# nextpyp/cet_pick

Measured on AMD Instinct MI355X. Metric: subtomograms/sec (MoCo-3D train) + voxels/sec (heatmap+NMS) at 1/2/4/8 GPU, higher is better.
Workload: dtype f32; 1 GPU; moco_main.py moco3d_18: 3D encoder, synthetic 512x512x128 tomogram, 32^3 subtomo crops, batch 64 per GPU, r=1024, dim=128, m=0.999, T=0.1, SGD lr 1e-3; global_batch=64, parallelism=dp1, hipgraph=True

## Files before the change

### cet_pick_amd/_lib.py

```python
import ctypes
import os

import torch

_HERE = os.path.dirname(os.path.abspath(__file__))
LIB_PATH = os.environ.get("CETPICK_HIP_LIB") or os.path.join(_HERE, "libcetpick_hip.so")

_c = ctypes
_P, _I, _F, _Z, _D, _L = _c.c_void_p, _c.c_int, _c.c_float, _c.c_size_t, _c.c_double, _c.c_long


class ConvGeom(ctypes.Structure):
    _fields_ = [(f, _I) for f in "N Di Hi Wi Ci Co kd kh kw stride pd ph pw dd dh dw".split()]


_G = _c.POINTER(ConvGeom)


class Aug2d3dRanges(ctypes.Structure):
    _fields_ = [(f, _F) for f in "flip_p angle_lo angle_hi erase_p scale_lo scale_hi ratio_lo ratio_hi".split()]


_R = _c.POINTER(Aug2d3dRanges)

# ... 10 lines not shown
    _fields_ = [(f, _I) for f in "P M R T label_dx label_dy glyph_px glyph_gap box_pad box_border".split()]


_PL = _c.POINTER(PlotLayout)

SIGNATURES = {
    "mi_abi_version": (_I, []),
    "mi_graph_node_counts": (_I, [_P, _P]),
    "mi_debug_stamp": (_I, [_P, _P]),
    "mi_linear_stats_fwd_f32": (_I, [_P] * 5 + [_I] * 3 + [_P]),
    "mi_debug_last_conv_kernel": (_c.c_char_p, []),
    "mi_debug_last_conv_plan": (_I, [_P, _I]),
    "mi_linear_bn_fwd_f32": (_I, [_P] * 5 + [_I] * 3 + [_P, _P, _F, _F] + [_P] * 4 + [_I, _P]),
    "mi_conv3d_stem_stats_workspace_bytes": (_Z, [_I] * 5),
    "mi_conv3d_stem_stats_f32": (_I, [_P, _P, _P] + [_I] * 5 + [_P, _P, _Z, _P]),
    "mi_build_arch": (_c.c_char_p, []),
    "mi_sigmoid_clamp": (_I, [_P, _P, _Z, _P]),
    "mi_nms3d": (_I, [_P, _P, _I, _I, _I, _I, _I, _P]),
    "mi_decode_workspace_bytes": (_Z, [_I, _I, _I, _I]),
    "mi_decode_workspace_init": (_I, [_P, _Z, _P]),
    "mi_sigmoid_nms_topk": (_I, [_P, _P, _I, _I, _I, _I, _I, _I, _I, _P, _P, _P, _Z, _P]),
    "mi_gauss3d_sep": (_I, [_P, _P, _P, _I, _I, _I, _F, _P]),
    "mi_dog_pick_workspace_bytes": (_Z, [_I, _I, _I, _I]),
    "mi_dog_pick": (_I, [_P, _I, _I, _I, _P, _I, _I, _I, _I, _P, _P, _P, _P, _I, _P, _P, _Z, _P]),
    "mi_greedy_nms3d_workspace_bytes": (_Z, [_I, _I, _I]),
    "mi_greedy_nms3d": (_I, [_P, _I, _I, _I, _F, _F, _F, _P, _P, _P, _I, _P, _Z, _P]),
    "mi_crop_normalize": (_I, [_P, _I, _I, _I, _P, _I, _I, _I, _I, _I, _I, _P, _P]),
    "mi_crop_normalize_table": (_I, [_P, _P, _P, _P, _P, _c.c_int64, _I, _I, _I, _I, _I, _I, _P, _P]),
    "mi_u8_roundtrip_normalize": (_I, [_P, _P, _Z, _F, _F, _P]),
    "mi_aug2d_params": (_I, [_P, _c.c_int64, _c.c_uint64, _I, _I, _I] + [_F] * 7 + [_P, _P]),
# ... 253 lines not shown
```

### cet_pick_amd/csrc/conv_igemm.hip

```cpp
#include "common.h"
#include "bf16x3.h"
#include <algorithm>
#include <cstdlib>
#include <type_traits>

int mi_stem7_fwd(const float* x, const float* w, float* y, const float* res, int relu, int N, int D, int H, int W,
                 int Co, int bf16x3, void* ws, size_t ws_bytes, hipStream_t s, double* sums = nullptr);
size_t mi_stem7_fwd_workspace_bytes();
size_t mi_stem7_fwd_stats_workspace_bytes(int N, int D, int H, int W);
size_t mi_stem7_wgrad_workspace_bytes(int N, int D, int H, int W, int Co);
int mi_stem7_wgrad(const float* x, const float* dy, float* dw, int N, int D, int H, int W, int Co, int bf16x3, void* ws,
                   size_t ws_bytes, hipStream_t s);

int mi_direct3_kind(int N, int Di, int Hi, int Wi, int Ci, int Co, int kd, int kh, int kw, int stride, int pd, int ph,
                    int pw, int dd, int dh, int dw);
size_t mi_direct3_wimg_bytes(int channels);
size_t mi_direct3_slab_bytes(int N, int channels);
int mi_direct3_prep(const float* const* w, void* const* img, const int* dgrad, const int* channels, int n, hipStream_t s);
int mi_direct3_launch(const float* a, const void* wimg, float* out, const float* res, const float* mask, int relu, int N,
                      int D, hipStream_t s);
size_t mi_direct3_wimg_bytes_kind(int kind);
int mi_direct3_prep_kind(const float* const* w, void* const* img, const int* dgrad, const int* kinds, int n, hipStream_t s);
int mi_direct3s_launch256(const float* a, const void* wimg, float* out, const float* res, const float* mask, int relu, int N,
                          hipStream_t s);
// ... 1227 lines not shown

extern "C" size_t mi_conv3d_stem_stats_workspace_bytes(int N, int Di, int Hi, int Wi, int Co) {
    Geom g = make_geom(N, Di, Hi, Wi, 1, Co, 7, 2, 3);
    if (!geom_ok(g) || !is_stem7(g) || Co != 64) return 0;
    return mi_stem7_fwd_stats_workspace_bytes(N, Di, Hi, Wi);
}

extern "C" int mi_conv3d_stem_stats_f32(const float* x, const float* w, float* y, int N, int Di, int Hi, int Wi, int Co,
                                        double* sums, void* ws, size_t ws_bytes, mi_stream_t stream) {
    Geom g = make_geom(N, Di, Hi, Wi, 1, Co, 7, 2, 3);
    if (!x || !w || !y || !sums || !geom_ok(g)) return MI_E_ARG;
    if (!is_stem7(g) || !conv_arith_bf16x3() || env_int("MI_CONV_NO_STEM") || env_int("MI_STEM_NO_STATS")) return MI_E_UNSUPPORTED;
    return mi_stem7_fwd(x, w, y, nullptr, 0, N, Di, Hi, Wi, Co, 1, ws, ws_bytes, (hipStream_t)stream, sums);
}

extern "C" int mi_linear_fwd_f32(const float* x, const float* w, const float* bias, float* y, int M, int Ci, int Co,
                                 void* ws, size_t ws_bytes, mi_stream_t stream) {
    Geom g = make_geom(M, 1, 1, 1, Ci, Co, 1, 1, 0);
    if (!x || !w || !y || !geom_ok(g)) return MI_E_ARG;
    return run_conv(MODE_FWD, g, x, w, y, bias, nullptr, 0, ws, ws_bytes, (hipStream_t)stream, nullptr, bias ? 1 : 0);
}

extern "C" int mi_conv_wgrad_batch_f32(const float* const* xs, const float* const* dys, float* const* dws, void* const* wss, int nb,
                                       const mi_conv_geom* pg, size_t ws_bytes, int* splits_out, mi_stream_t stream) {
    Geom g;
    if (!xs || !dys || !dws || !wss || !splits_out || nb < 1 || !public_geom(pg, &g)) return MI_E_ARG;
    for (int i = 0; i < nb; ++i) if (!xs[i] || !dys[i] || !dws[i]) return MI_E_ARG;
    if (nb < 2 || !conv_arith_bf16x3() || env_int("MI_NO_WGRAD_BATCH")) return MI_E_UNSUPPORTED;
    hipStream_t s = (hipStream_t)stream;
    float* slabs[MI_WGRAD_BATCH_MAX];
// ... 82 lines not shown
```

### cet_pick_amd/csrc/conv_stem.hip

```cpp
#include "common.h"
#include "bf16x3.h"
#include <type_traits>
#include "../../include/cetpick_hip.h"

namespace {

using namespace bf3;

constexpr int K7 = 7, S2 = 2, P3 = 3;
constexpr int TX = 8, TY = 4, TZ = 4;
constexpr int PX = S2 * (TX - 1) + K7;
constexpr int PY = S2 * (TY - 1) + K7;
constexpr int PZ = S2 * (TZ - 1) + K7;
constexpr int PW = 24;
constexpr int PATCH = PZ * PY * PW;
constexpr int KS = 50;
constexpr int WS = 64;
constexpr int WROWS = 64;
constexpr int CO = 64;

struct StemParams {
    const float* x;
    const float* w;
    float* y;
    const float* res;
    int relu;
    int N, D, H, W, Do, Ho, Wo;
    unsigned x_bytes;
    double* stats;
};

__global__ __launch_bounds__(256) void stem_fwd_kernel(StemParams p) {
    constexpr int NP = (PATCH + PW + 255) / 256;
    __shared__ __attribute__((aligned(16))) float patch[NP * 256];
    __shared__ __attribute__((aligned(16))) float wl[2][WROWS * WS];
    const int tid = threadIdx.x, lane = tid & 63, wave = tid >> 6;
    const int h = lane >> 5, l32 = lane & 31;
    const int txn = p.Wo / TX, tyn = p.Ho / TY, tzn = p.Do / TZ;
    int b = blockIdx.x;
    const int bx = b % txn; b /= txn;
    const int by = b % tyn; b /= tyn;
    const int bz = b % tzn;
    const int n = b / tzn;
    const int ox0 = bx * TX, oy0 = by * TY, oz0 = bz * TZ;
// ... 93 lines not shown
constexpr int WSLAB = 3 * WPL;
constexpr size_t WPREP_BYTES = (size_t)K7 * WSLAB;

__global__ __launch_bounds__(256) void stem_wprep_kernel(const float* w, unsigned short* out) {
    const int i = blockIdx.x * 256 + threadIdx.x;
    if (i >= K7 * 8 * CO * 8) return;
    const int kx = i & 7, co = (i >> 3) & (CO - 1), j = (i >> 9) & 7, slab = i >> 12;
    const int r = 8 * slab + j, kz = r / K7, ky = r % K7;
    const float v = (r < K7 * K7 && kx < K7) ? w[((kz * K7 + ky) * K7 + kx) * CO + co] : 0.f;
    unsigned h0, h1, h2;
    cut3(v, h0, h1, h2);
    const int o = slab * (WSLAB / 2) + (j * CO + co) * 8 + kx;
    out[o] = (unsigned short)h0; out[o + WPL / 2] = (unsigned short)h1; out[o + WPL] = (unsigned short)h2;
}

template <int NBUF, int ZPW>
__global__ __launch_bounds__(256, ZPW == 2 ? 2 : (NBUF == 1 ? 3 : 2)) void stem_fwd_bf3_kernel(StemParams p, const unsigned char* wprep) {
    constexpr int TZ = 4 * ZPW;
    constexpr int PZ = S2 * (TZ - 1) + K7;
    constexpr int PPLANE = PZ * PYP * PROW;
    __shared__ __attribute__((aligned(16))) unsigned char patchb[3 * PPLANE];
    __shared__ __attribute__((aligned(16))) unsigned char wl[NBUF][WSLAB];
    const int tid = threadIdx.x, lane = tid & 63, wave = tid >> 6;
    const int h = lane >> 5, l32 = lane & 31;
    const int txn = p.Wo / TX, tyn = p.Ho / TY, tzn = p.Do / TZ;
    int b = blockIdx.x;
    const int bx = b % txn; b /= txn;
    const int by = b % tyn; b /= tyn;
    const int bz = b % tzn;
    const int n = b / tzn;
    const int ox0 = bx * TX, oy0 = by * TY, oz0 = bz * TZ;

// ... 123 lines not shown
            frags(sl + 1, 0, S0{}, nextTail);
        } else {
            frags(sl + 1, 0, S0{}, nextTail);
            __builtin_amdgcn_sched_barrier(0);
            mfmas(S1{});
        }
    };
    __syncthreads();
    frags(0, 0, S0{}, NoTail{});
    for (int sl = 0; sl < K7 - 2; ++sl) slab_body(sl, NoTail{});
    slab_body(K7 - 2, Tail{});
    __builtin_amdgcn_sched_barrier(0);
    mfmas(S0{});

    float cs[2][2];
#pragma unroll
    for (int j = 0; j < 2; ++j) {
        const int co = j * 32 + l32;
        float t0 = 0.f, t1 = 0.f;
#pragma unroll
        for (int zi = 0; zi < ZPW; ++zi) {
            const int oz = oz0 + ZPW * wave + zi;
#pragma unroll
            for (int r = 0; r < 16; ++r) {
                const int m = (r & 3) + 8 * (r >> 2) + 4 * h;
                const int ox = ox0 + (m & 7), oy = oy0 + (m >> 3);
                const long o = ((((long)n * p.Do + oz) * p.Ho + oy) * p.Wo + ox) * CO + co;
                float v = j == 0 ? acc0[zi][r] : acc1[zi][r];
                if (p.res) v += p.res[o];
                if (p.relu) v = fmaxf(v, 0.f);
                p.y[o] = v;
                t0 += v; t1 = fmaf(v, v, t1);
            }
        }
        cs[j][0] = t0; cs[j][1] = t1;
    }
    if (p.stats) {
        float* red = reinterpret_cast<float*>(patchb);
#pragma unroll
        for (int j = 0; j < 2; ++j)
#pragma unroll
            for (int q = 0; q < 2; ++q) {
                const float o = cs[j][q] + __shfl_xor(cs[j][q], 32);
                if (h == 0) red[(wave * 2 + q) * CO + j * 32 + l32] = o;
            }
        __syncthreads();
        if (tid < 2 * CO) {
            const int q = tid >> 6, c = tid & (CO - 1);
            double a = 0;
#pragma unroll
            for (int w = 0; w < 4; ++w) a += (double)red[(w * 2 + q) * CO + c];
            p.stats[(long)(q * CO + c) * gridDim.x + blockIdx.x] = a;
        }
    }
}

__global__ __launch_bounds__(256) void stem_stats_finalize_kernel(const double* part, int n_part, double* sums) {
    __shared__ double red[256];
    const double* src = part + (long)blockIdx.x * n_part;
    double a = 0;
    for (int i = threadIdx.x; i < n_part; i += 256) a += src[i];
    red[threadIdx.x] = a;
    __syncthreads();
#pragma unroll
    for (int o = 128; o > 0; o >>= 1) {
        if ((int)threadIdx.x < o) red[threadIdx.x] += red[threadIdx.x + o];
        __syncthreads();
    }
// ... 366 lines not shown
        MI_RETURN_IF_LAUNCH_FAILED();
        const bool z8 = Do % (2 * TZ) == 0 && !getenv("MI_STEM_FWD_Z4") && !getenv("MI_STEM_FWD_NBUF2");
        const long nb = z8 ? blocks / 2 : blocks;
        if (z8) hipLaunchKernelGGL((stem_fwd_bf3_kernel<1, 2>), dim3((unsigned)nb), dim3(256), 0, s, p, (const unsigned char*)ws);
        else if (getenv("MI_STEM_FWD_NBUF2")) hipLaunchKernelGGL((stem_fwd_bf3_kernel<2, 1>), dim3((unsigned)blocks), dim3(256), 0, s, p, (const unsigned char*)ws);
        else hipLaunchKernelGGL((stem_fwd_bf3_kernel<1, 1>), dim3((unsigned)blocks), dim3(256), 0, s, p, (const unsigned char*)ws);
        MI_RETURN_IF_LAUNCH_FAILED();
        if (sums) {
            hipLaunchKernelGGL(stem_stats_finalize_kernel, dim3(2 * CO), dim3(256), 0, s, (const double*)p.stats, (int)nb,
                               sums);
            MI_RETURN_IF_LAUNCH_FAILED();
        }
        return MI_OK;
    }
    hipLaunchKernelGGL(stem_fwd_kernel, dim3((unsigned)blocks), dim3(256), 0, s, p);
    MI_RETURN_IF_LAUNCH_FAILED();
    return MI_OK;
}

constexpr int RED_GROUPS = 32;

static int stem7_wgrad_blocks(long tiles) {
    long b = tiles < 512 ? tiles : 512;
    return (int)b;
}

size_t mi_stem7_wgrad_workspace_bytes(int N, int D, int H, int W, int Co) {
    if (Co != CO) return 0;
    const int Do = (D + 2 * P3 - K7) / S2 + 1, Ho = (H + 2 * P3 - K7) / S2 + 1, Wo = (W + 2 * P3 - K7) / S2 + 1;
    if (Do <= 0 || Ho <= 0 || Wo <= 0 || Do % TZ || Ho % TY || Wo % TX) return 0;
// ... 34 lines not shown
```

### cet_pick_amd/csrc/train_ops.hip

```cpp
#include "common.h"
#include "bf16x3.h"
#include <algorithm>

namespace {

using bf3::ld4;
using bf3::st4;

enum { CR_STATS = 0, CR_BNBWD = 1, CR_SUM = 2, CR_BNBWD_X = 3 };

struct PoolGeom { int N, Di, Hi, Wi, Do, Ho, Wo, k, s, pad; };

struct ColReduceParams {
    const float* a;
    const float* x;
    const float* y;
    const float* save;
    long M;
    int C, relu;
    double* partials;
    const float* gamma;
    const float* beta;
    double* sums_direct;
    float* f32_direct;
// ... 133 lines not shown
struct BnStat4 { float mean[4], inv[4]; double var[4]; };
__device__ __forceinline__ BnStat4 bn_stat4(const double* sums, double count, int C, int c, float eps) {
    BnStat4 r;
#pragma unroll
    for (int k = 0; k < 4; ++k) {
        const double mean = sums[c + k] / count;
        double var = sums[C + c + k] / count - mean * mean;
        if (var < 0) var = 0;
        r.mean[k] = (float)mean;
        r.inv[k] = (float)(1.0 / sqrt(var + (double)eps));
        r.var[k] = var;
    }
    return r;
}

__global__ __launch_bounds__(256) void bn_apply_kernel(const float* x, float* y, long n4, int C,
                                                      const double* sums, double count, float eps,
                                                      float momentum, float* running_mean,
                                                      float* running_var, long long* num_batches_tracked,
                                                      float* save, const float* gamma,
                                                      const float* beta, const float* res, int relu) {
    const int CV = C >> 2;
    const int c = (int)(threadIdx.x % CV) * 4;
    float m[4], iv[4];
    if (sums) {
        const BnStat4 st = bn_stat4(sums, count, C, c, eps);
#pragma unroll
        for (int k = 0; k < 4; ++k) { m[k] = st.mean[k]; iv[k] = st.inv[k]; }
        if (blockIdx.x == 0 && threadIdx.x < CV) {
#pragma unroll
            for (int k = 0; k < 4; ++k) {
                if (save) { save[c + k] = m[k]; save[C + c + k] = iv[k]; }
                if (running_mean) {
                    const double unbiased = count > 1 ? st.var[k] * count / (count - 1.0) : st.var[k];
                    running_mean[c + k] = (1.f - momentum) * running_mean[c + k] + momentum * m[k];
                    running_var[c + k] = (1.f - momentum) * running_var[c + k] + momentum * (float)unbiased;
                }
            }
            if (threadIdx.x == 0 && num_batches_tracked) *num_batches_tracked += 1;
        }
    } else {
#pragma unroll
        for (int k = 0; k < 4; ++k) { m[k] = running_mean[c + k]; iv[k] = 1.0f / sqrtf(running_var[c + k] + eps); }
        if (save && blockIdx.x == 0 && threadIdx.x < CV) {
#pragma unroll
            for (int k = 0; k < 4; ++k) { save[c + k] = m[k]; save[C + c + k] = iv[k]; }
        }
    }
    const float4 g = gamma ? ld4(gamma + c) : make_float4(1, 1, 1, 1);
    const float4 b = beta ? ld4(beta + c) : make_float4(0, 0, 0, 0);
    for (long i = (long)blockIdx.x * 256 + threadIdx.x; i < n4; i += (long)gridDim.x * 256) {
        float4 v = ld4(x + 4 * i);
        float4 o;
        o.x = fmaf((v.x - m[0]) * iv[0], g.x, b.x); o.y = fmaf((v.y - m[1]) * iv[1], g.y, b.y);
        o.z = fmaf((v.z - m[2]) * iv[2], g.z, b.z); o.w = fmaf((v.w - m[3]) * iv[3], g.w, b.w);
// ... 3 lines not shown
    }
}

__global__ __launch_bounds__(256) void bn_relu_maxpool_fwd_kernel(const float* x, float* y, uint8_t* arg, PoolGeom g,
                                                                 int C, const double* sums, double count, float eps,
                                                                 float momentum, float* running_mean,
                                                                 float* running_var, long long* num_batches_tracked,
                                                                 float* save, const float* gamma, const float* beta) {
    const int CV = C >> 2;
    const int c = (int)(threadIdx.x % CV) * 4;
    float m[4], iv[4];
    if (sums) {
        const BnStat4 st = bn_stat4(sums, count, C, c, eps);
#pragma unroll
        for (int k = 0; k < 4; ++k) { m[k] = st.mean[k]; iv[k] = st.inv[k]; }
        if (blockIdx.x == 0 && threadIdx.x < CV) {
#pragma unroll
            for (int k = 0; k < 4; ++k) {
                if (save) { save[c + k] = m[k]; save[C + c + k] = iv[k]; }
                if (running_mean) {
                    const double unbiased = count > 1 ? st.var[k] * count / (count - 1.0) : st.var[k];
                    running_mean[c + k] = (1.f - momentum) * running_mean[c + k] + momentum * m[k];
                    running_var[c + k] = (1.f - momentum) * running_var[c + k] + momentum * (float)unbiased;
                }
            }
            if (threadIdx.x == 0 && num_batches_tracked) *num_batches_tracked += 1;
        }
    } else {
#pragma unroll
        for (int k = 0; k < 4; ++k) { m[k] = running_mean[c + k]; iv[k] = 1.0f / sqrtf(running_var[c + k] + eps); }
    }
    const float4 g4 = gamma ? ld4(gamma + c) : make_float4(1, 1, 1, 1);
    const float4 b4 = beta ? ld4(beta + c) : make_float4(0, 0, 0, 0);
    const float gg[4] = {g4.x, g4.y, g4.z, g4.w}, bb[4] = {b4.x, b4.y, b4.z, b4.w};
    const long total = (long)g.N * g.Do * g.Ho * g.Wo * CV;
    for (long i = (long)blockIdx.x * 256 + threadIdx.x; i < total; i += (long)gridDim.x * 256) {
        unsigned v = (unsigned)i / (unsigned)CV;
        const int xo = (int)(v % (unsigned)g.Wo); v /= (unsigned)g.Wo;
        const int yo = (int)(v % (unsigned)g.Ho); v /= (unsigned)g.Ho;
        const int zo = (int)(v % (unsigned)g.Do);
        const int n = (int)(v / (unsigned)g.Do);
        float best[4] = {-INFINITY, -INFINITY, -INFINITY, -INFINITY};
// ... 39 lines not shown
                    const float4 t4 = ld4(x + ((((long)n * g.Di + zi) * g.Hi + yi) * g.Wi + xi) * C + c);
                    const float xv[4] = {t4.x, t4.y, t4.z, t4.w};
                    const int tap = (a * g.k + b) * g.k + cc;
#pragma unroll
                    for (int q = 0; q < 4; ++q) {
                        const float t = fmaxf(fmaf((xv[q] - m[q]) * iv[q], gg[q], bb[q]), 0.f);
                        const float tn = xv[q] != xv[q] ? xv[q] : t;
                        if (first || tn > best[q] || tn != tn) { best[q] = tn; bi[q] = tap; }
                    }
                    first = false;
                }
            }
        }
        st4(y + 4 * i, make_float4(best[0], best[1], best[2], best[3]));
        if (arg) *reinterpret_cast<uchar4*>(arg + 4 * i) = make_uchar4(bi[0], bi[1], bi[2], bi[3]);
    }
}

__global__ __launch_bounds__(256) void bn_relu_bwd_apply_x_kernel(const float* dy, const float* x, float* dx, long n4, int C,
                                                                 const float* save, const float* gamma, const float* beta,
                                                                 const double* sums, double count, float* dgamma,
                                                                 float* dbeta) {
    const int CV = C >> 2;
    const int c = (int)(threadIdx.x % CV) * 4;
    const float rc = (float)(1.0 / count);
    float mean[4], inv[4], gi[4], gg[4], bb[4], sdy[4], sdx[4];
#pragma unroll
    for (int k = 0; k < 4; ++k) {
        mean[k] = save[c + k]; inv[k] = save[C + c + k];
        gg[k] = gamma ? gamma[c + k] : 1.f; bb[k] = beta ? beta[c + k] : 0.f;
// ... 654 lines not shown
                                        float* running_mean, float* running_var, long long* num_batches_tracked,
                                        float* save_mean_invstd, mi_stream_t stream) {
    PoolGeom g;
    if (!x || !y || !colreduce_ok(C) || !pool_geom(N, Di, Hi, Wi, k, stride, pad, &g)) return MI_E_ARG;
    if (sums ? (!save_mean_invstd || !(count > 0)) : (!running_mean || !running_var)) return MI_E_ARG;
    if ((running_mean == nullptr) != (running_var == nullptr)) return MI_E_ARG;
    const long total = (long)N * g.Do * g.Ho * g.Wo * (C / 4);
    if (total >= (1l << 31)) return MI_E_UNSUPPORTED;
    hipLaunchKernelGGL(bn_relu_maxpool_fwd_kernel, dim3(ew_blocks(total)), dim3(256), 0, (hipStream_t)stream, x, y, argmax,
                       g, C, sums, count, eps, momentum, running_mean, running_var, num_batches_tracked,
                       save_mean_invstd, gamma, beta);
    MI_RETURN_IF_LAUNCH_FAILED();
    return MI_OK;
}

extern "C" int mi_bn_relu_bwd_reduce_x(const float* dy, const float* x, long M, int C, const float* save_mean_invstd,
                                       const float* gamma, const float* beta, double* sums, void* ws, size_t ws_bytes,
                                       mi_stream_t stream) {
    if (!dy || !x || !save_mean_invstd || !sums) return MI_E_ARG;
    ColReduceParams p = {};
    p.a = dy; p.x = x; p.save = save_mean_invstd; p.M = M; p.C = C; p.gamma = gamma; p.beta = beta;
    return run_colreduce<CR_BNBWD_X>(p, sums, ws, ws_bytes, (hipStream_t)stream);
}

extern "C" int mi_bn_relu_bwd_apply_x(const float* dy, const float* x, float* dx, long M, int C,
                                      const float* save_mean_invstd, const float* gamma, const float* beta,
                                      const double* sums, double count, float* dgamma, float* dbeta, mi_stream_t stream) {
    if (!dy || !x || !dx || !save_mean_invstd || !sums || !colreduce_ok(C) || M <= 0 || !(count > 0)) return MI_E_ARG;
    const long n4 = M * C / 4;
    hipLaunchKernelGGL(bn_relu_bwd_apply_x_kernel, dim3(ew_blocks(n4)), dim3(256), 0, (hipStream_t)stream, dy, x, dx, n4, C,
// ... 428 lines not shown
```

### cet_pick_amd/hipops.py

```python
import collections
import ctypes
import math
import os
import torch
import torch.nn as nn

from . import _lib as L


PROFILE = None
PROFILE_REPEAT = 8


def _prof_run(tag, flops, fn):
    fn()
    if PROFILE is not None:
        e0 = torch.cuda.Event(enable_timing=True)
        e1 = torch.cuda.Event(enable_timing=True)
        e0.record()
        for _ in range(PROFILE_REPEAT):
            fn()
        e1.record()
        PROFILE.append((tag, flops, e0, e1, PROFILE_REPEAT))

# ... 898 lines not shown
    if nbytes == 0:
        return None
    do, ho, wo = [(v + 6 - 7) // 2 + 1 for v in (d, h, wd)]
    y = torch.empty((n, do, ho, wo, co), dtype=torch.float32, device=x.device)
    sums = torch.empty(2 * co, dtype=torch.float64, device=x.device)
    ws = _ws(nbytes, x.device, "stem_stats")
    rc = lib.mi_conv3d_stem_stats_f32(L.ptr(x), L.ptr(w), L.ptr(y), n, d, h, wd, co, L.ptr(sums), L.ptr(ws), ws.numel(),
                                      L.stream())
    if rc == -3:
        return None
    L.check(rc, "mi_conv3d_stem_stats_f32")
    mod.bn_sums = sums
    return y


class GradSlot:
    __slots__ = ("tensor",)

    def __init__(self):
        self.tensor = None


FUSE_RES_GRAD = os.environ.get("CETPICK_FUSE_RES_GRAD", "1") != "0"


def grad_slot_for(x):
    return GradSlot() if (FUSE_RES_GRAD and torch.is_grad_enabled() and x.requires_grad and x.is_cuda and PROFILE is None) else None


class _ConvFn(torch.autograd.Function):
# ... 1483 lines not shown
```

### cet_pick_amd/models/networks/moco_encoder_3d.py

```python
import torch
import torch.nn as nn

from ... import hipops as H

BN_MOMENTUM = 0.1


def fill_fc_weights(layers):
    for m in layers.modules():
        if isinstance(m, H.HipConv3d):
            nn.init.normal_(m.weight, std=0.001)
        elif isinstance(m, H.HipLinear):
            nn.init.normal_(m.weight, std=0.001)
            if m.bias is not None:
                nn.init.constant_(m.bias, 0.001)


class BasicBlock(nn.Module):
    expansion = 1

    def __init__(self, inplanes, planes, stride=1, dilation=1, downsample=None):
        super().__init__()
        if dilation != 1:
            raise NotImplementedError("dilation != 1 is not used by the moco3d encoder")
# ... 47 lines not shown
            layers.append(block(self.inplanes, planes, dilation=dilation))
        return nn.Sequential(*layers)

    grad_marker = None

    def _mark(self, x, tag):
        if self.grad_marker is not None and x.requires_grad:
            x.register_hook(lambda g, t=tag: self.grad_marker(t))
        return x

    def _trunk(self, x1):
        b, c, d, h, w = x1.shape
        if c != 1:
            raise ValueError("the moco3d encoder takes single-channel sub-tomograms (B,1,D,H,W)")
        x = x1.contiguous().float().view(b, d, h, w, 1)
        self.conv1.stats_for_bn = self.bn1.training or not self.bn1.track_running_stats
        x = self.conv1(x)
        sums = getattr(self.conv1, "bn_sums", None) if self.conv1.stats_for_bn else None
        self.conv1.bn_sums = None
        H.stamp("stem")
        x = self._mark(H.bn_relu_maxpool3d(x, self.bn1, 3, 2, 1, sums=sums), "layer1")
        H.stamp("pool")
        first = True
        for tag, layer in (("layer2", self.layer1), ("layer3", self.layer2), (None, self.layer3)):
            for blk in layer:
                x = blk(x, mask_dx=not first, dout_masked=True)
                first = False
            if tag is not None:
                x = self._mark(x, tag)
            H.stamp("layer")
        x = self.feature_3d[0](x, mask_dx=True)
        if H.RELU_TAP is not None:
            import copy
            with torch.no_grad():
                H.RELU_TAP["feature_3d"] = copy.deepcopy(self.feature_3d[1])(x.detach(), relu=True).clone()
        x = H.bn_relu_global_avgpool(x, self.feature_3d[1])
# ... 3 lines not shown
        seq = self.__getattr__(head)
        H.stamp("trunk")
        x = H.linear_bn(x, seq[0], seq[1], relu=True)
        if H.RELU_TAP is not None:
            H.RELU_TAP[head + ".1"] = x.detach().clone()
        x = H.linear_bn(x, seq[3], seq[4], relu=True)
        if H.RELU_TAP is not None:
            H.RELU_TAP[head + ".4"] = x.detach().clone()
        return H.linear_bn(x, seq[6], seq[7])

    def forward_sync_gen(self, x1):
        b, c, d, h, w = x1.shape
        if c != 1:
            raise ValueError("the moco3d encoder takes single-channel sub-tomograms (B,1,D,H,W)")
        x = x1.contiguous().float().view(b, d, h, w, 1)
        self.conv1.stats_for_bn = True
        x = self.conv1(x)
        sums = getattr(self.conv1, "bn_sums", None)
        self.conv1.bn_sums = None
        if sums is None:
            sums = H.bn_local_sums(x)
        yield sums
        x = self._mark(H.bn_relu_maxpool3d(x, self.bn1, 3, 2, 1, sums=sums, reduced=True), "layer1")
        first = True
        for tag, layer in (("layer2", self.layer1), ("layer3", self.layer2), (None, self.layer3)):
            for blk in layer:
                x = blk(x, mask_dx=not first, dout_masked=True)
                first = False
            if tag is not None:
                x = self._mark(x, tag)
        x = self.feature_3d[0](x, mask_dx=True)
        sums = H.bn_local_sums(x)
        yield sums
        x = H.global_avgpool(self.feature_3d[1](x, relu=True, sums=sums, reduced=True))
        x = self.fc(x)
        ret1 = {}
        for head in self.heads:
            if "proj" in head:
# ... 48 lines not shown
```

### include/cetpick_hip.h

```cpp
#ifndef CETPICK_HIP_H
#define CETPICK_HIP_H

#include <stddef.h>
#include <stdint.h>

#ifdef __cplusplus
extern "C" {
#endif

typedef void* mi_stream_t;

#define MI_OK 0
#define MI_E_ARG (-1)
#define MI_E_WORKSPACE (-2)
#define MI_E_UNSUPPORTED (-3)

int mi_abi_version(void);
int mi_graph_node_counts(void* graph, int* counts);
int mi_debug_stamp(void* slot, mi_stream_t stream);
const char* mi_debug_last_conv_kernel(void);
int mi_debug_last_conv_plan(int* out, int n);
const char* mi_build_arch(void);


// ... 193 lines not shown
size_t mi_zhead_bwd_workspace_bytes(int N, int D, long P, int C, int K);
int mi_zhead_bwd(const float* x, const float* w, const float* dy, float* dx, float* dw, int N, int D, long P, int C,
                 int K, void* ws, size_t ws_bytes, mi_stream_t stream);

size_t mi_colreduce_workspace_bytes(long M, int C);
int mi_bn_stats(const float* x, long M, int C, double* sums, void* ws, size_t ws_bytes,
                mi_stream_t stream);
int mi_bn_apply_fwd(const float* x, float* y, long M, int C, const double* sums, double count,
                    const float* gamma, const float* beta, float eps, float momentum,
                    float* running_mean, float* running_var, long long* num_batches_tracked,
                    float* save_mean_invstd, const float* res, int relu, mi_stream_t stream);
int mi_bn_relu_maxpool3d_fwd(const float* x, float* y, uint8_t* argmax, int N, int Di, int Hi, int Wi, int C, int k,
                             int stride, int pad, const double* sums, double count, const float* gamma,
                             const float* beta, float eps, float momentum, float* running_mean, float* running_var,
                             long long* num_batches_tracked, float* save_mean_invstd, mi_stream_t stream);
int mi_bn_relu_bwd_reduce_x(const float* dy, const float* x, long M, int C, const float* save_mean_invstd,
                            const float* gamma, const float* beta, double* sums, void* ws, size_t ws_bytes,
                            mi_stream_t stream);
int mi_bn_relu_bwd_apply_x(const float* dy, const float* x, float* dx, long M, int C, const float* save_mean_invstd,
                           const float* gamma, const float* beta, const double* sums, double count, float* dgamma,
                           float* dbeta, mi_stream_t stream);
#define MI_BN_SMALL_MAX_ROWS 4096
int mi_bn_small_fwd(const float* x, float* y, long M, int C, const float* gamma, const float* beta, float eps,
                    float momentum, float* running_mean, float* running_var, long long* num_batches_tracked,
                    float* save_mean_invstd, const float* res, int relu, mi_stream_t stream);
int mi_bn_small_bwd(const float* dy, const float* x, const float* y, float* dx, long M, int C,
                    const float* save_mean_invstd, const float* gamma, int relu, float* dgamma, float* dbeta,
                    mi_stream_t stream);
int mi_bn_small_pool_fwd(const float* x, float* y, float* pooled, long M, int C, int V, const float* gamma,
                         const float* beta, float eps, float momentum, float* running_mean, float* running_var,
// ... 179 lines not shown
```

Before: 41650 subtomograms/sec.

## Fuse max-pool pre-reduction into the stem conv epilogue for no-grad forward

Result: no change. 41560 subtomograms/sec (-0.2%).

```diff
diff --git a/cet_pick_amd/_lib.py b/cet_pick_amd/_lib.py
--- a/cet_pick_amd/_lib.py
+++ b/cet_pick_amd/_lib.py
@@ -48,6 +48,9 @@
     "mi_linear_bn_fwd_f32": (_I, [_P] * 5 + [_I] * 3 + [_P, _P, _F, _F] + [_P] * 4 + [_I, _P]),
     "mi_conv3d_stem_stats_workspace_bytes": (_Z, [_I] * 5),
     "mi_conv3d_stem_stats_f32": (_I, [_P, _P, _P] + [_I] * 5 + [_P, _P, _Z, _P]),
+    "mi_conv3d_stem_pool_slab_bytes": (_Z, [_I] * 5),
+    "mi_conv3d_stem_pool_f32": (_I, [_P, _P, _P] + [_I] * 5 + [_P, _P, _Z, _P, _Z, _P]),
+    "mi_stem_pool_finish_fwd": (_I, [_P, _Z, _P] + [_I] * 5 + [_P, _D, _P, _P, _F, _F] + [_P] * 5),
     "mi_build_arch": (_c.c_char_p, []),
     "mi_sigmoid_clamp": (_I, [_P, _P, _Z, _P]),
     "mi_nms3d": (_I, [_P, _P, _I, _I, _I, _I, _I, _P]),
diff --git a/cet_pick_amd/csrc/conv_igemm.hip b/cet_pick_amd/csrc/conv_igemm.hip
--- a/cet_pick_amd/csrc/conv_igemm.hip
+++ b/cet_pick_amd/csrc/conv_igemm.hip
@@ -8,6 +8,9 @@
                  int Co, int bf16x3, void* ws, size_t ws_bytes, hipStream_t s, double* sums = nullptr);
 size_t mi_stem7_fwd_workspace_bytes();
 size_t mi_stem7_fwd_stats_workspace_bytes(int N, int D, int H, int W);
+size_t mi_stem7_fwd_pool_slab_bytes(int N, int D, int H, int W);
+int mi_stem7_fwd_pool(const float* x, const float* w, const float* gamma, int N, int D, int H, int W, int Co, void* ws,
+                      size_t ws_bytes, void* slab, size_t slab_bytes, hipStream_t s, double* sums);
 size_t mi_stem7_wgrad_workspace_bytes(int N, int D, int H, int W, int Co);
 int mi_stem7_wgrad(const float* x, const float* dy, float* dw, int N, int D, int H, int W, int Co, int bf16x3, void* ws,
                    size_t ws_bytes, hipStream_t s);
@@ -1265,6 +1268,20 @@
     return mi_stem7_fwd(x, w, y, nullptr, 0, N, Di, Hi, Wi, Co, 1, ws, ws_bytes, (hipStream_t)stream, sums);
 }
 
+extern "C" size_t mi_conv3d_stem_pool_slab_bytes(int N, int Di, int Hi, int Wi, int Co) {
+    Geom g = make_geom(N, Di, Hi, Wi, 1, Co, 7, 2, 3);
+    if (!geom_ok(g) || !is_stem7(g) || Co != 64) return 0;
+    return mi_stem7_fwd_pool_slab_bytes(N, Di, Hi, Wi);
+}
+
+extern "C" int mi_conv3d_stem_pool_f32(const float* x, const float* w, const float* gamma, int N, int Di, int Hi, int Wi, int Co,
+                                       double* sums, void* slab, size_t slab_bytes, void* ws, size_t ws_bytes, mi_stream_t stream) {
+    Geom g = make_geom(N, Di, Hi, Wi, 1, Co, 7, 2, 3);
+    if (!x || !w || !sums || !slab || !geom_ok(g)) return MI_E_ARG;
+    if (!is_stem7(g) || !conv_arith_bf16x3() || env_int("MI_CONV_NO_STEM") || env_int("MI_STEM_NO_STATS")) return MI_E_UNSUPPORTED;
+    return mi_stem7_fwd_pool(x, w, gamma, N, Di, Hi, Wi, Co, ws, ws_bytes, slab, slab_bytes, (hipStream_t)stream, sums);
+}
+
 extern "C" int mi_linear_fwd_f32(const float* x, const float* w, const float* bias, float* y, int M, int Ci, int Co,
                                  void* ws, size_t ws_bytes, mi_stream_t stream) {
     Geom g = make_geom(M, 1, 1, 1, Ci, Co, 1, 1, 0);
diff --git a/cet_pick_amd/csrc/conv_stem.hip b/cet_pick_amd/csrc/conv_stem.hip
--- a/cet_pick_amd/csrc/conv_stem.hip
+++ b/cet_pick_amd/csrc/conv_stem.hip
@@ -1,5 +1,6 @@
 #include "common.h"
 #include "bf16x3.h"
+#include "stem_pool.h"
 #include <type_traits>
 #include "../../include/cetpick_hip.h"
 
@@ -28,6 +29,8 @@
     int N, D, H, W, Do, Ho, Wo;
     unsigned x_bytes;
     double* stats;
+    int* pool;
+    const float* pool_gamma;
 };
 
 __global__ __launch_bounds__(256) void stem_fwd_kernel(StemParams p) {
@@ -151,8 +154,9 @@
     out[o] = (unsigned short)h0; out[o + WPL / 2] = (unsigned short)h1; out[o + WPL] = (unsigned short)h2;
 }
 
-template <int NBUF, int ZPW>
+template <int NBUF, int ZPW, bool POOL = false>
 __global__ __launch_bounds__(256, ZPW == 2 ? 2 : (NBUF == 1 ? 3 : 2)) void stem_fwd_bf3_kernel(StemParams p, const unsigned char* wprep) {
+    static_assert(!POOL || ZPW == 2, "the pooled epilogue is written for the 8 x 4 x 8 tile");
     constexpr int TZ = 4 * ZPW;
     constexpr int PZ = S2 * (TZ - 1) + K7;
     constexpr int PPLANE = PZ * PYP * PROW;
@@ -306,26 +310,64 @@
     mfmas(S0{});
 
     float cs[2][2];
+    int wk[POOL ? 2 : 1][3][3], uk[POOL ? 2 : 1][3][3];
 #pragma unroll
     for (int j = 0; j < 2; ++j) {
         const int co = j * 32 + l32;
         float t0 = 0.f, t1 = 0.f;
+        [[maybe_unused]] const unsigned flip = POOL ? stem_pool::flip_of(p.pool_gamma, co) : 0u;
 #pragma unroll
         for (int zi = 0; zi < ZPW; ++zi) {
             const int oz = oz0 + ZPW * wave + zi;
+            [[maybe_unused]] int key[16];
 #pragma unroll
             for (int r = 0; r < 16; ++r) {
                 const int m = (r & 3) + 8 * (r >> 2) + 4 * h;
                 const int ox = ox0 + (m & 7), oy = oy0 + (m >> 3);
-                const long o = ((((long)n * p.Do + oz) * p.Ho + oy) * p.Wo + ox) * CO + co;
+                [[maybe_unused]] const long o = ((((long)n * p.Do + oz) * p.Ho + oy) * p.Wo + ox) * CO + co;
                 float v = j == 0 ? acc0[zi][r] : acc1[zi][r];
-                if (p.res) v += p.res[o];
-                if (p.relu) v = fmaxf(v, 0.f);
-                p.y[o] = v;
+                if constexpr (POOL) {
+                    key[r] = stem_pool::key_of(v, flip);
+                } else {
+                    if (p.res) v += p.res[o];
+                    if (p.relu) v = fmaxf(v, 0.f);
+                    p.y[o] = v;
+                }
                 t0 += v; t1 = fmaf(v, v, t1);
             }
+            if constexpr (POOL) {
+                int xs[4][3];
+#pragma unroll
+                for (int y = 0; y < 4; ++y) {
+                    const int a0 = key[4 * y], a1 = key[4 * y + 1], a2 = key[4 * y + 2], a3 = key[4 * y + 3];
+                    const int m01 = max(a0, a1), m123 = max(a1, max(a2, a3));
+                    const int part = h ? m01 : a3;
+                    xs[y][0] = h ? m123 : m01;
+                    xs[y][1] = h ? a3 : m123;
+                    xs[y][2] = max(part, __shfl_xor(part, 32));
+                }
+#pragma unroll
+                for (int sx = 0; sx < 3; ++sx) {
+                    const int y0 = max(xs[0][sx], xs[1][sx]), y1 = max(xs[1][sx], max(xs[2][sx], xs[3][sx])), y2 = xs[3][sx];
+                    if (zi == 0) { wk[j][0][sx] = y0; wk[j][1][sx] = y1; wk[j][2][sx] = y2; }
+                    else {
+                        uk[j][0][sx] = y0; uk[j][1][sx] = y1; uk[j][2][sx] = y2;
+                        wk[j][0][sx] = max(wk[j][0][sx], y0); wk[j][1][sx] = max(wk[j][1][sx], y1); wk[j][2][sx] = max(wk[j][2][sx], y2);
+                    }
+                }
+            }
         }
         cs[j][0] = t0; cs[j][1] = t1;
+    }
+    if constexpr (POOL) {
+        int* ex = reinterpret_cast<int*>(patchb + 2048);
+        __syncthreads();
+        if (wave < 3) {
+#pragma unroll
+            for (int j = 0; j < 2; ++j)
+#pragma unroll
+                for (int q = 0; q < 9; ++q) ex[((wave * 2 + j) * 9 + q) * 64 + lane] = uk[j][q / 3][q % 3];
+        }
     }
     if (p.stats) {
         float* red = reinterpret_cast<float*>(patchb);
@@ -344,6 +386,24 @@
             for (int w = 0; w < 4; ++w) a += (double)red[(w * 2 + q) * CO + c];
             p.stats[(long)(q * CO + c) * gridDim.x + blockIdx.x] = a;
         }
+    }
+    if constexpr (POOL) {
+        if (!p.stats) __syncthreads();
+        const int* ex = reinterpret_cast<const int*>(patchb + 2048);
+        int* dst = p.pool + (size_t)blockIdx.x * stem_pool::TILE_KEYS;
+#pragma unroll
+        for (int j = 0; j < 2; ++j)
+#pragma unroll
+            for (int q = 0; q < 9; ++q) {
+                const int qy = q / 3, sx = q % 3;
+                if (sx == 2 && h) continue;
+                const int qx = h ? 3 + sx : sx;
+                int v = wk[j][qy][sx];
+                if (wave > 0) v = max(v, ex[(((wave - 1) * 2 + j) * 9 + q) * 64 + lane]);
+                dst[((wave * stem_pool::QY + qy) * stem_pool::QX + qx) * CO + j * 32 + l32] = v;
+                if (wave == 3)
+                    dst[((4 * stem_pool::QY + qy) * stem_pool::QX + qx) * CO + j * 32 + l32] = uk[j][qy][sx];
+            }
     }
 }
 
@@ -740,6 +800,35 @@
         return MI_OK;
     }
     hipLaunchKernelGGL(stem_fwd_kernel, dim3((unsigned)blocks), dim3(256), 0, s, p);
+    MI_RETURN_IF_LAUNCH_FAILED();
+    return MI_OK;
+}
+
+size_t mi_stem7_fwd_pool_slab_bytes(int N, int D, int H, int W) {
+    const int Do = (D + 2 * P3 - K7) / S2 + 1, Ho = (H + 2 * P3 - K7) / S2 + 1, Wo = (W + 2 * P3 - K7) / S2 + 1;
+    if (N <= 0 || Do <= 0 || Ho <= 0 || Wo <= 0 || Do % (2 * TZ) || Ho % TY || Wo % TX) return 0;
+    return sizeof(int) * stem_pool::TILE_KEYS * ((size_t)N * (Do / (2 * TZ)) * (Ho / TY) * (Wo / TX));
+}
+
+int mi_stem7_fwd_pool(const float* x, const float* w, const float* gamma, int N, int D, int H, int W, int Co, void* ws,
+                      size_t ws_bytes, void* slab, size_t slab_bytes, hipStream_t s, double* sums) {
+    static_assert(TX == 2 * stem_pool::HX && TY == 2 * stem_pool::HY && 2 * TZ == 2 * stem_pool::HZ && CO == stem_pool::CH, "stem_pool.h");
+    if (Co != CO || !sums || !ws || !slab) return MI_E_UNSUPPORTED;
+    const size_t need = mi_stem7_fwd_pool_slab_bytes(N, D, H, W);
+    if (need == 0 || slab_bytes < need || getenv("MI_STEM_FWD_Z4") || getenv("MI_STEM_FWD_NBUF2")) return MI_E_UNSUPPORTED;
+    if (ws_bytes < mi_stem7_fwd_stats_workspace_bytes(N, D, H, W)) return MI_E_UNSUPPORTED;
+    const int Do = (D + 2 * P3 - K7) / S2 + 1, Ho = (H + 2 * P3 - K7) / S2 + 1, Wo = (W + 2 * P3 - K7) / S2 + 1;
+    const long xb = 4l * N * D * H * W;
+    if (xb >= 0x7fff0000l) return MI_E_UNSUPPORTED;
+    const long nb = (long)N * (Do / (2 * TZ)) * (Ho / TY) * (Wo / TX);
+    if (nb > 0x3fffffffl) return MI_E_UNSUPPORTED;
+    StemParams p = {x, w, nullptr, nullptr, 0, N, D, H, W, Do, Ho, Wo, (unsigned)xb, nullptr, (int*)slab, gamma};
+    p.stats = reinterpret_cast<double*>((unsigned char*)ws + ((WPREP_BYTES + 255) & ~(size_t)255));
+    hipLaunchKernelGGL(stem_wprep_kernel, dim3((K7 * 8 * CO * 8 + 255) / 256), dim3(256), 0, s, w, (unsigned short*)ws);
+    MI_RETURN_IF_LAUNCH_FAILED();
+    hipLaunchKernelGGL((stem_fwd_bf3_kernel<1, 2, true>), dim3((unsigned)nb), dim3(256), 0, s, p, (const unsigned char*)ws);
+    MI_RETURN_IF_LAUNCH_FAILED();
+    hipLaunchKernelGGL(stem_stats_finalize_kernel, dim3(2 * CO), dim3(256), 0, s, (const double*)p.stats, (int)nb, sums);
     MI_RETURN_IF_LAUNCH_FAILED();
     return MI_OK;
 }
diff --git a/cet_pick_amd/csrc/stem_pool.h b/cet_pick_amd/csrc/stem_pool.h
--- /dev/null
+++ b/cet_pick_amd/csrc/stem_pool.h
@@ -0,0 +1,22 @@
+#pragma once
+
+namespace stem_pool {
+
+constexpr int QX = 5, QY = 3, QZ = 5;
+constexpr int HX = 4, HY = 2, HZ = 4;
+constexpr int CH = 64;
+constexpr int TILE_KEYS = QZ * QY * QX * CH;
+constexpr int KEY_NAN = 0x7fffffff;
+
+__device__ __forceinline__ int key_of(float v, unsigned flip) {
+    const int k = (int)(__float_as_uint(v) ^ flip);
+    return v != v ? KEY_NAN : (k >= 0 ? k : k ^ 0x7fffffff);
+}
+__device__ __forceinline__ float value_of(int k, unsigned flip) {
+    return __uint_as_float((unsigned)(k >= 0 ? k : k ^ 0x7fffffff) ^ flip);
+}
+__device__ __forceinline__ unsigned flip_of(const float* gamma, int c) {
+    return (gamma && !(gamma[c] >= 0.f)) ? 0x80000000u : 0u;
+}
+
+}
diff --git a/cet_pick_amd/csrc/train_ops.hip b/cet_pick_amd/csrc/train_ops.hip
--- a/cet_pick_amd/csrc/train_ops.hip
+++ b/cet_pick_amd/csrc/train_ops.hip
@@ -1,5 +1,7 @@
 #include "common.h"
 #include "bf16x3.h"
+#include "stem_pool.h"
+#include <climits>
 #include <algorithm>
 
 namespace {
@@ -171,6 +173,20 @@
     return r;
 }
 
+__device__ __forceinline__ void bn_track4(const BnStat4& st, int c, int C, double count, float momentum, float* running_mean,
+                                          float* running_var, long long* num_batches_tracked, float* save) {
+#pragma unroll
+    for (int k = 0; k < 4; ++k) {
+        if (save) { save[c + k] = st.mean[k]; save[C + c + k] = st.inv[k]; }
+        if (running_mean) {
+            const double unbiased = count > 1 ? st.var[k] * count / (count - 1.0) : st.var[k];
+            running_mean[c + k] = (1.f - momentum) * running_mean[c + k] + momentum * st.mean[k];
+            running_var[c + k] = (1.f - momentum) * running_var[c + k] + momentum * (float)unbiased;
+        }
+    }
+    if (threadIdx.x == 0 && num_batches_tracked) *num_batches_tracked += 1;
+}
+
 __global__ __launch_bounds__(256) void bn_apply_kernel(const float* x, float* y, long n4, int C,
                                                       const double* sums, double count, float eps,
                                                       float momentum, float* running_mean,
@@ -184,18 +200,8 @@
         const BnStat4 st = bn_stat4(sums, count, C, c, eps);
 #pragma unroll
         for (int k = 0; k < 4; ++k) { m[k] = st.mean[k]; iv[k] = st.inv[k]; }
-        if (blockIdx.x == 0 && threadIdx.x < CV) {
-#pragma unroll
-            for (int k = 0; k < 4; ++k) {
-                if (save) { save[c + k] = m[k]; save[C + c + k] = iv[k]; }
-                if (running_mean) {
-                    const double unbiased = count > 1 ? st.var[k] * count / (count - 1.0) : st.var[k];
-                    running_mean[c + k] = (1.f - momentum) * running_mean[c + k] + momentum * m[k];
-                    running_var[c + k] = (1.f - momentum) * running_var[c + k] + momentum * (float)unbiased;
-                }
-            }
-            if (threadIdx.x == 0 && num_batches_tracked) *num_batches_tracked += 1;
-        }
+        if (blockIdx.x == 0 && threadIdx.x < CV)
+            bn_track4(st, c, C, count, momentum, running_mean, running_var, num_batches_tracked, save);
     } else {
 #pragma unroll
         for (int k = 0; k < 4; ++k) { m[k] = running_mean[c + k]; iv[k] = 1.0f / sqrtf(running_var[c + k] + eps); }
@@ -229,18 +235,8 @@
         const BnStat4 st = bn_stat4(sums, count, C, c, eps);
 #pragma unroll
         for (int k = 0; k < 4; ++k) { m[k] = st.mean[k]; iv[k] = st.inv[k]; }
-        if (blockIdx.x == 0 && threadIdx.x < CV) {
-#pragma unroll
-            for (int k = 0; k < 4; ++k) {
-                if (save) { save[c + k] = m[k]; save[C + c + k] = iv[k]; }
-                if (running_mean) {
-                    const double unbiased = count > 1 ? st.var[k] * count / (count - 1.0) : st.var[k];
-                    running_mean[c + k] = (1.f - momentum) * running_mean[c + k] + momentum * m[k];
-                    running_var[c + k] = (1.f - momentum) * running_var[c + k] + momentum * (float)unbiased;
-                }
-            }
-            if (threadIdx.x == 0 && num_batches_tracked) *num_batches_tracked += 1;
-        }
+        if (blockIdx.x == 0 && threadIdx.x < CV)
+            bn_track4(st, c, C, count, momentum, running_mean, running_var, num_batches_tracked, save);
     } else {
 #pragma unroll
         for (int k = 0; k < 4; ++k) { m[k] = running_mean[c + k]; iv[k] = 1.0f / sqrtf(running_var[c + k] + eps); }
@@ -310,6 +306,50 @@
         }
         st4(y + 4 * i, make_float4(best[0], best[1], best[2], best[3]));
         if (arg) *reinterpret_cast<uchar4*>(arg + 4 * i) = make_uchar4(bi[0], bi[1], bi[2], bi[3]);
+    }
+}
+
+__global__ __launch_bounds__(256) void stem_pool_finish_kernel(const int* slab, float* y, int N, int Do, int Ho, int Wo,
+                                                              const double* sums, double count, float eps, float momentum,
+                                                              float* running_mean, float* running_var,
+                                                              long long* num_batches_tracked, float* save, const float* gamma,
+                                                              const float* beta) {
+    using namespace stem_pool;
+    constexpr int C = CH, CV = CH >> 2;
+    const int c = (int)(threadIdx.x % CV) * 4;
+    const BnStat4 st = bn_stat4(sums, count, C, c, eps);
+    if (blockIdx.x == 0 && threadIdx.x < CV)
+        bn_track4(st, c, C, count, momentum, running_mean, running_var, num_batches_tracked, save);
+    const float4 g4 = gamma ? ld4(gamma + c) : make_float4(1, 1, 1, 1);
+    const float4 b4 = beta ? ld4(beta + c) : make_float4(0, 0, 0, 0);
+    const float gg[4] = {g4.x, g4.y, g4.z, g4.w}, bb[4] = {b4.x, b4.y, b4.z, b4.w};
+    const int txn = Wo / HX, tyn = Ho / HY, tzn = Do / HZ;
+    const long total = (long)N * Do * Ho * Wo * CV;
+    for (long i = (long)blockIdx.x * 256 + threadIdx.x; i < total; i += (long)gridDim.x * 256) {
+        unsigned v = (unsigned)i / (unsigned)CV;
+        const int xo = (int)(v % (unsigned)Wo); v /= (unsigned)Wo;
+        const int yo = (int)(v % (unsigned)Ho); v /= (unsigned)Ho;
+        const int zo = (int)(v % (unsigned)Do);
+        const int n = (int)(v / (unsigned)Do);
+        const int bx = xo / HX, qx = xo % HX, by = yo / HY, qy = yo % HY, bz = zo / HZ, qz = zo % HZ;
+        int4 best = make_int4(INT_MIN, INT_MIN, INT_MIN, INT_MIN);
+        for (int dz = 0; dz <= (qz == 0 && bz > 0); ++dz)
+            for (int dy = 0; dy <= (qy == 0 && by > 0); ++dy)
+                for (int dx = 0; dx <= (qx == 0 && bx > 0); ++dx) {
+                    const long tile = (((long)n * tzn + (bz - dz)) * tyn + (by - dy)) * txn + (bx - dx);
+                    const int wz = dz ? QZ - 1 : qz, wy = dy ? QY - 1 : qy, wx = dx ? QX - 1 : qx;
+                    const int4 k = *reinterpret_cast<const int4*>(slab + tile * TILE_KEYS + ((wz * QY + wy) * QX + wx) * CH + c);
+                    best.x = max(best.x, k.x); best.y = max(best.y, k.y); best.z = max(best.z, k.z); best.w = max(best.w, k.w);
+                }
+        const int kk[4] = {best.x, best.y, best.z, best.w};
+        float o[4];
+#pragma unroll
+        for (int r = 0; r < 4; ++r) {
+            const float xv = value_of(kk[r], gg[r] >= 0.f ? 0u : 0x80000000u);
+            const float t = fmaxf(fmaf((xv - st.mean[r]) * st.inv[r], gg[r], bb[r]), 0.f);
+            o[r] = xv != xv ? xv : t;
+        }
+        st4(y + 4 * i, make_float4(o[0], o[1], o[2], o[3]));
     }
 }
 
@@ -994,6 +1034,25 @@
     return MI_OK;
 }
 
+extern "C" int mi_stem_pool_finish_fwd(const void* slab, size_t slab_bytes, float* y, int N, int Do, int Ho, int Wo, int C,
+                                       const double* sums, double count, const float* gamma, const float* beta, float eps,
+                                       float momentum, float* running_mean, float* running_var, long long* num_batches_tracked,
+                                       float* save_mean_invstd, mi_stream_t stream) {
+    using namespace stem_pool;
+    if (!slab || !y || !sums || !save_mean_invstd || !(count > 0) || N <= 0 || Do <= 0 || Ho <= 0 || Wo <= 0) return MI_E_ARG;
+    if ((running_mean == nullptr) != (running_var == nullptr)) return MI_E_ARG;
+    if (C != CH || Do % HZ || Ho % HY || Wo % HX) return MI_E_UNSUPPORTED;
+    const long tiles = (long)N * (Do / HZ) * (Ho / HY) * (Wo / HX);
+    if (slab_bytes < sizeof(int) * (size_t)TILE_KEYS * (size_t)tiles) return MI_E_WORKSPACE;
+    const long total = (long)N * Do * Ho * Wo * (C / 4);
+    if (total >= (1l << 31)) return MI_E_UNSUPPORTED;
+    hipLaunchKernelGGL(stem_pool_finish_kernel, dim3(ew_blocks(total)), dim3(256), 0, (hipStream_t)stream, (const int*)slab, y, N,
+                       Do, Ho, Wo, sums, count, eps, momentum, running_mean, running_var, num_batches_tracked, save_mean_invstd,
+                       gamma, beta);
+    MI_RETURN_IF_LAUNCH_FAILED();
+    return MI_OK;
+}
+
 extern "C" int mi_bn_relu_bwd_reduce_x(const float* dy, const float* x, long M, int C, const float* save_mean_invstd,
                                        const float* gamma, const float* beta, double* sums, void* ws, size_t ws_bytes,
                                        mi_stream_t stream) {
diff --git a/cet_pick_amd/hipops.py b/cet_pick_amd/hipops.py
--- a/cet_pick_amd/hipops.py
+++ b/cet_pick_amd/hipops.py
@@ -936,6 +936,48 @@
     return y
 
 
+STEM_POOL_FUSED = os.environ.get("CETPICK_STEM_POOL_FUSED", "1") != "0"
+
+
+def stem_conv_pooled(x, conv, bn):
+    w = conv.weight
+    needs_grad = torch.is_grad_enabled() and any(t is not None and t.requires_grad for t in (x, w, bn.weight, bn.bias))
+    if (not STEM_POOL_FUSED or needs_grad or PROFILE is not None or not (bn.training or not bn.track_running_stats)
+            or not x.is_cuda or x.dtype != torch.float32 or x.dim() != 5 or x.shape[-1] != 1 or not x.is_contiguous()
+            or (conv.k, conv.stride, conv.pad) != (7, 2, 3) or not _phys_ok(w) or getattr(conv, "dil", None) is not None):
+        return None
+    lib = L.lib()
+    n, d, h, wd, _ = x.shape
+    co = w.shape[0]
+    nslab = lib.mi_conv3d_stem_pool_slab_bytes(n, d, h, wd, co)
+    nbytes = lib.mi_conv3d_stem_stats_workspace_bytes(n, d, h, wd, co)
+    if nslab == 0 or nbytes == 0:
+        return None
+    slab = _ws(nslab, x.device, "stem_pool_slab")
+    ws = _ws(nbytes, x.device, "stem_stats")
+    sums = torch.empty(2 * co, dtype=torch.float64, device=x.device)
+    rc = lib.mi_conv3d_stem_pool_f32(L.ptr(x), L.ptr(w), L.ptr(bn.weight), n, d, h, wd, co, L.ptr(sums), L.ptr(slab), slab.numel(),
+                                     L.ptr(ws), ws.numel(), L.stream())
+    if rc == -3:
+        return None
+    L.check(rc, "mi_conv3d_stem_pool_f32")
+    return slab, sums, (n,) + tuple((v + 6 - 7) // 2 + 1 for v in (d, h, wd)) + (co,)
+
+
+def stem_pool_finish(part, bn, reduced=False):
+    slab, sums, (n, d, h, w, c) = part
+    y = torch.empty((n, d // 2, h // 2, w // 2, c), dtype=torch.float32, device=slab.device)
+    save = torch.empty(2 * c, dtype=torch.float32, device=slab.device)
+    sums, count = _bn_batch_sums(None, n * d * h * w, c, bn, sums, reduced)
+    track = bn.track_running_stats and bn.training
+    running_mean, running_var, _ = _bn_running_ptrs(bn, track)
+    L.check(L.lib().mi_stem_pool_finish_fwd(
+        L.ptr(slab), slab.numel(), L.ptr(y), n, d // 2, h // 2, w // 2, c, L.ptr(sums), count, L.ptr(bn.weight), L.ptr(bn.bias),
+        bn.eps, bn.momentum, running_mean, running_var, L.ptr(bn.num_batches_tracked if track else None), L.ptr(save),
+        L.stream()), "mi_stem_pool_finish_fwd")
+    return y
+
+
 class GradSlot:
     __slots__ = ("tensor",)
 
diff --git a/cet_pick_amd/models/networks/moco_encoder_3d.py b/cet_pick_amd/models/networks/moco_encoder_3d.py
--- a/cet_pick_amd/models/networks/moco_encoder_3d.py
+++ b/cet_pick_amd/models/networks/moco_encoder_3d.py
@@ -85,12 +85,17 @@
         if c != 1:
             raise ValueError("the moco3d encoder takes single-channel sub-tomograms (B,1,D,H,W)")
         x = x1.contiguous().float().view(b, d, h, w, 1)
-        self.conv1.stats_for_bn = self.bn1.training or not self.bn1.track_running_stats
-        x = self.conv1(x)
-        sums = getattr(self.conv1, "bn_sums", None) if self.conv1.stats_for_bn else None
-        self.conv1.bn_sums = None
-        H.stamp("stem")
-        x = self._mark(H.bn_relu_maxpool3d(x, self.bn1, 3, 2, 1, sums=sums), "layer1")
+        part = H.stem_conv_pooled(x, self.conv1, self.bn1)
+        if part is not None:
+            H.stamp("stem")
+            x = H.stem_pool_finish(part, self.bn1)
+        else:
+            self.conv1.stats_for_bn = self.bn1.training or not self.bn1.track_running_stats
+            x = self.conv1(x)
+            sums = getattr(self.conv1, "bn_sums", None) if self.conv1.stats_for_bn else None
+            self.conv1.bn_sums = None
+            H.stamp("stem")
+            x = self._mark(H.bn_relu_maxpool3d(x, self.bn1, 3, 2, 1, sums=sums), "layer1")
         H.stamp("pool")
         first = True
         for tag, layer in (("layer2", self.layer1), ("layer3", self.layer2), (None, self.layer3)):
@@ -124,14 +129,19 @@
         if c != 1:
             raise ValueError("the moco3d encoder takes single-channel sub-tomograms (B,1,D,H,W)")
         x = x1.contiguous().float().view(b, d, h, w, 1)
-        self.conv1.stats_for_bn = True
-        x = self.conv1(x)
-        sums = getattr(self.conv1, "bn_sums", None)
-        self.conv1.bn_sums = None
-        if sums is None:
-            sums = H.bn_local_sums(x)
-        yield sums
-        x = self._mark(H.bn_relu_maxpool3d(x, self.bn1, 3, 2, 1, sums=sums, reduced=True), "layer1")
+        part = H.stem_conv_pooled(x, self.conv1, self.bn1)
+        if part is not None:
+            yield part[1]
+            x = H.stem_pool_finish(part, self.bn1, reduced=True)
+        else:
+            self.conv1.stats_for_bn = True
+            x = self.conv1(x)
+            sums = getattr(self.conv1, "bn_sums", None)
+            self.conv1.bn_sums = None
+            if sums is None:
+                sums = H.bn_local_sums(x)
+            yield sums
+            x = self._mark(H.bn_relu_maxpool3d(x, self.bn1, 3, 2, 1, sums=sums, reduced=True), "layer1")
         first = True
         for tag, layer in (("layer2", self.layer1), ("layer3", self.layer2), (None, self.layer3)):
             for blk in layer:
diff --git a/include/cetpick_hip.h b/include/cetpick_hip.h
--- a/include/cetpick_hip.h
+++ b/include/cetpick_hip.h
@@ -231,6 +231,13 @@
                              int stride, int pad, const double* sums, double count, const float* gamma,
                              const float* beta, float eps, float momentum, float* running_mean, float* running_var,
                              long long* num_batches_tracked, float* save_mean_invstd, mi_stream_t stream);
+size_t mi_conv3d_stem_pool_slab_bytes(int N, int Di, int Hi, int Wi, int Co);
+int mi_conv3d_stem_pool_f32(const float* x, const float* w, const float* gamma, int N, int Di, int Hi, int Wi, int Co,
+                            double* sums, void* slab, size_t slab_bytes, void* ws, size_t ws_bytes, mi_stream_t stream);
+int mi_stem_pool_finish_fwd(const void* slab, size_t slab_bytes, float* y, int N, int Do, int Ho, int Wo, int C,
+                            const double* sums, double count, const float* gamma, const float* beta, float eps, float momentum,
+                            float* running_mean, float* running_var, long long* num_batches_tracked, float* save_mean_invstd,
+                            mi_stream_t stream);
 int mi_bn_relu_bwd_reduce_x(const float* dy, const float* x, long M, int C, const float* save_mean_invstd,
                             const float* gamma, const float* beta, double* sums, void* ws, size_t ws_bytes,
                             mi_stream_t stream);
```
